# pharaofranz/frb-baseband

Measured on NVIDIA B200. Metric: input baseband GB/s (VDIF bytes, headers included) per B200, 2 Gbps 16x32 MHz 2-bit -> 8-bit Stokes I, higher is better.
Workload: dtype f32

## Files before the change

### frb-baseband_b200/csrc/b2f_api.cu

```cuda
#include <cuda_runtime.h>

#include <algorithm>
#include <cmath>
#include <cstdio>
#include <cstdlib>
#include <cstring>
#include <numeric>
#include <string>
#include <vector>

#define B2F_API_TU
#include "b2f_fused.cuh"
#include "b2f_generic.cuh"
#include "b2f_launch.h"

using namespace b2f;

namespace {

thread_local std::string g_err;

int fail(int code, const std::string& msg) {
    g_err = msg;
    return code;
// ... 57 lines not shown
    bool generic = false;
    int tsq = 1;
    float* d_Fk = nullptr;
    int64_t Fk_if_stride = 0, fk_pending = 0;
    int kgt_lg = 0;
    int kgt_cols = 0, kgt_rb = 0, kgt_col_ctas = 0, kgt_row_ctas = 0;
    bool carry_mode = false;
    float2 *d_tw_col = nullptr, *d_tw_row = nullptr;
    int nfilt_pos = 0, nfilt_neg = 0, keep = 0;
    int64_t step = 0;
    int64_t carry_len = 0;
    uint8_t* d_carry = nullptr;
    int bps = 1;
    bool smask = false;
    uint8_t* d_carry_mask = nullptr;
    float4* d_levels_stream = nullptr;
    int64_t levels_stride = 0;
    float2* d_spec = nullptr;
    float2* d_chirp = nullptr;
    uint8_t* d_out_stage[2]{};
    size_t out_stage_bytes[2]{};
    int path = 0;
    uint8_t* d_tstream = nullptr;  size_t tstream_stride = 0;
    int* d_fillflag = nullptr;     size_t fillflag_stride = 0;
    float* d_part = nullptr;       int64_t part_if_stride = 0;
    int Dp = 0;
    unsigned* d_fsync = nullptr;
    int f_grid = 0, f_lanes = 0, f_nslot = 3, f_lag = 2;
    bool f_aborted = false;
    float4* d_levels = nullptr;
    unsigned long long* d_fprof = nullptr;

    int64_t rows_base = 0;
    int64_t rows_off = 0;
    int64_t rows_held = 0;
    int64_t rows_produced = 0, rows_emitted = 0;
    bool stats_ready = false, flushed = false, have_base = false;
    int64_t rows_this_interval = 0;
    bool preset_stats = false;
    int64_t frames_pushed = 0;
    uint32_t base_sec0[B2F_MAX_IF]{}, base_fnum0[B2F_MAX_IF]{};
    int64_t last_nblk = 0, last_nframes = 0;
    unsigned long long blocks_dirty = 0;

    std::vector<TimedLaunch> pending;
    std::vector<std::pair<cudaEvent_t, cudaEvent_t>> ev_pool;
// ... 155 lines not shown
    body();
    CU(cudaGetLastError());
    return 0;
}

void free_plan(b2f_plan* pl) {
    if (!pl) return;
    cudaSetDevice(pl->prm.device);
    cudaDeviceSynchronize();
    for (int i = 0; i < 2; ++i) {
        if (pl->d_stage[i]) cudaFree(pl->d_stage[i]);
        if (pl->ev_stage_free[i]) cudaEventDestroy(pl->ev_stage_free[i]);
        if (pl->ev_h2d_done[i]) cudaEventDestroy(pl->ev_h2d_done[i]);
        if (pl->ev_out_free[i]) cudaEventDestroy(pl->ev_out_free[i]);
        if (pl->ev_kq_done[i]) cudaEventDestroy(pl->ev_kq_done[i]);
        if (pl->d_out_stage[i]) cudaFree(pl->d_out_stage[i]);
    }
    for (int i = 0; i < b2f_plan::kMarks; ++i)
        for (int k = 0; k < 3; ++k)
            if (pl->ev_mark[i][k]) cudaEventDestroy(pl->ev_mark[i][k]);
    void* bufs[] = {pl->d_compact, pl->d_wmask, pl->d_fstat, pl->d_blkdirty, pl->d_inter, pl->d_colsum,
                    pl->d_eps, pl->d_F, pl->d_mean, pl->d_scale, pl->d_partial, pl->d_tab_g, pl->d_tab_h,
                    pl->d_tab_w, pl->d_tab_r, pl->d_tab_beta, pl->d_counters, pl->d_carry, pl->d_spec, pl->d_chirp, pl->d_tw_col, pl->d_tw_row,
                    pl->d_tstream, pl->d_fillflag, pl->d_part, pl->d_fsync, pl->d_fprof, pl->d_levels, pl->d_carry_mask, pl->d_levels_stream};
    for (void* b : bufs)
        if (b) cudaFree(b);
    if (pl->d_Fk) cudaFree(pl->d_Fk);
    for (auto& t : pl->pending) { cudaEventDestroy(t.a); cudaEventDestroy(t.b); }
    for (auto& e : pl->ev_pool) { cudaEventDestroy(e.first); cudaEventDestroy(e.second); }
    if (pl->copy_stream) cudaStreamDestroy(pl->copy_stream);
    if (pl->d2h_stream) cudaStreamDestroy(pl->d2h_stream);
    if (pl->own_stream && pl->stream) cudaStreamDestroy(pl->stream);
    delete pl;
}

int init_state(b2f_plan* pl) {
    pl->rows_base = pl->rows_off = pl->rows_held = pl->rows_produced = pl->rows_emitted = 0;
    pl->stats_ready = pl->prm.keep_bandpass != 0 || pl->preset_stats;
    pl->flushed = false;
    pl->have_base = false;
    pl->frames_pushed = 0;
    pl->carry_len = 0;
    pl->fk_pending = 0;
    pl->blocks_dirty = 0;
    pl->last_nblk = pl->last_nframes = 0;
    pl->rows_this_interval = 0;
    pl->f_aborted = false;
// ... 258 lines not shown
    }
    if (pl->f_aborted) return fail(B2F_ECUDA, "fused channeliser: inter-warp wait timed out (results of this scan are invalid)");
    return 0;
}

int push_fused(b2f_plan* pl, const K0Params& k0, int64_t nframes, int64_t nblk) {
    const int nif = pl->prm.nif;
    const int64_t nbt = (int64_t)nif * nblk;
    int rc = 0;
    for (int i = 0; i < nif; ++i)
        if (reinterpret_cast<uintptr_t>(k0.frames[i]) & 15) return fail(B2F_EINVAL, "frames must be 16-byte aligned");
    K0HParams kh{};
    K0TParams kt{};
    for (int i = 0; i < nif; ++i) {
        kh.frames[i] = k0.frames[i]; kt.frames[i] = k0.frames[i];
        kh.base_sec[i] = k0.base_sec[i]; kh.base_fnum[i] = k0.base_fnum[i];
    }
    kh.fstat = pl->d_fstat; kh.fstat_stride = pl->fstat_stride; kh.counters = pl->d_counters;
    kh.nframes = nframes; kh.frame_bytes = pl->prm.frame_bytes; kh.header_bytes = pl->prm.header_bytes;
    kh.in_nbit = pl->prm.in_nbit; kh.fps = (int)pl->fps; kh.nif = nif;
    kt.fstat = pl->d_fstat; kt.fstat_stride = pl->fstat_stride;
    kt.fillflag = pl->d_fillflag; kt.fillflag_stride = pl->fillflag_stride;
    kt.tstream = pl->d_tstream; kt.tstream_if_stride = pl->tstream_stride; kt.counters = pl->d_counters;
    kt.nblk = (int)nblk; kt.nif = nif; kt.R = pl->R; kt.frame_bytes = pl->prm.frame_bytes;
    kt.header_bytes = pl->prm.header_bytes; kt.payload_bytes = (int)pl->payload; kt.mask_faults = pl->prm.mask_faults;
    CU(cudaMemsetAsync(pl->d_fillflag, 0, pl->fillflag_stride * nif * sizeof(int), pl->stream));
    rc = timed(pl, B2F_K_VALIDATE, [&] {
        const int64_t n = nframes * nif;
        k0h_headers<<<(unsigned)((n + 255) / 256), 256, 0, pl->stream>>>(kh);
        if (nblk > 0) {
            const int sc = std::min(64, pl->R);
            const int64_t units = nbt * (pl->R / sc);
            const unsigned grid = (unsigned)std::min<int64_t>(units, (int64_t)pl->num_sms * (sc == 64 ? 6 : 8));
            if (sc == 64) k0t_transpose<64><<<grid, 256, 0, pl->stream>>>(kt);
            else if (sc == 32) k0t_transpose<32><<<grid, 256, 0, pl->stream>>>(kt);
            else k0t_transpose<16><<<grid, 256, 0, pl->stream>>>(kt);
        }
    });
    if (rc) return rc;
    pl->launches++;
    if (nblk == 0) return 0;
    if (pl->d_levels) {
        KJParams kj{};
        for (int i = 0; i < nif; ++i) kj.frames[i] = k0.frames[i];
        kj.fstat = pl->d_fstat; kj.fstat_stride = pl->fstat_stride; kj.levels = pl->d_levels;
        kj.nblk = (int)nblk; kj.nif = nif; kj.R = pl->R; kj.frame_bytes = pl->prm.frame_bytes;
        kj.header_bytes = pl->prm.header_bytes; kj.payload_bytes = (int)pl->payload; kj.mask_faults = pl->prm.mask_faults;
        const int64_t nthreads = nbt * pl->R * 32;
        rc = timed(pl, B2F_K_VALIDATE, [&] { kj_ja98_levels<<<(unsigned)((nthreads + 255) / 256), 256, 0, pl->stream>>>(kj); });
        if (rc) return rc;
    }

    FParams fp{};
    fp.tstream = pl->d_tstream; fp.tstream_if_stride = pl->tstream_stride;
    fp.ring = pl->d_inter; fp.colsum = pl->d_colsum; fp.eps = pl->d_eps;
    fp.tab_h = pl->d_tab_h; fp.tab_w = pl->d_tab_w; fp.tab_beta = pl->d_tab_beta; fp.tab_r = pl->d_tab_r;
    const bool direct = pl->Dp == pl->D || pl->path == 1;
    fp.out = direct ? row_dst(pl) : pl->d_part;
    fp.out_if_stride = direct ? row_dst_stride(pl) : pl->part_if_stride;
    fp.out_row0 = direct ? row_dst_row0(pl) : 0;
    fp.Dp = pl->Dp; fp.nblk = (int)nblk; fp.nif = nif;
    fp.gb_begin = 0; fp.gb_end = nbt;
    fp.sync = pl->d_fsync; fp.abort_flag = pl->d_fsync + (size_t)pl->f_lanes * FS_STRIDE;
    fp.nslot = pl->f_nslot; fp.lag = pl->f_lag; fp.prof = pl->d_fprof; fp.levels = pl->d_levels;
    cudaError_t e = cudaSuccess;
    if (pl->path == 2) {
        CU(cudaMemsetAsync(pl->d_fsync, 0, (size_t)pl->f_lanes * FS_STRIDE * sizeof(unsigned), pl->stream));
        fp.phase = 0;
        rc = timed(pl, B2F_K_FUSED, [&] { e = b2f_launch_kf(pl->R, pl->prm.pol_mode, fp, pl->f_grid, 1, pl->stream, nullptr); });
        if (rc) return rc;
        if (e != cudaSuccess) return fail(B2F_ECUDA, std::string("fused channeliser launch: ") + cudaGetErrorString(e));
    } else {
        fp.phase = 1;
        rc = timed(pl, B2F_K_COLUMN, [&] { e = b2f_launch_kf(pl->R, B2F_POL_I, fp, pl->f_grid, 0, pl->stream, nullptr); });
        if (rc) return rc;
        if (e != cudaSuccess) return fail(B2F_ECUDA, std::string("column half launch: ") + cudaGetErrorString(e));
        rc = timed(pl, B2F_K_EPS, [&] {
// ... 279 lines not shown
    } else {
        CUB(cudaStreamCreateWithFlags(&pl->stream, cudaStreamNonBlocking));
        pl->own_stream = true;
    }
    CUB(cudaStreamCreateWithFlags(&pl->copy_stream, cudaStreamNonBlocking));
    CUB(cudaStreamCreateWithFlags(&pl->d2h_stream, cudaStreamNonBlocking));
    for (int i = 0; i < 2; ++i) {
        CUB(cudaEventCreateWithFlags(&pl->ev_stage_free[i], cudaEventDisableTiming));
        CUB(cudaEventCreateWithFlags(&pl->ev_h2d_done[i], cudaEventDisableTiming));
        CUB(cudaEventCreateWithFlags(&pl->ev_out_free[i], cudaEventDisableTiming));
        CUB(cudaEventCreateWithFlags(&pl->ev_kq_done[i], cudaEventDisableTiming));
    }
    const int nif = prm->nif;
    const int64_t nbt = (int64_t)nif * pl->chunk_blocks;
    pl->slot_bytes = W ? (int)spf : (prm->in_nbit == 8 ? payload : (int)spf);
    pl->compact_stride = (size_t)((pl->chunk_frames * (int64_t)pl->slot_bytes + (pl->carry_mode ? pl->M * pl->bps : 0) + 255) / 256 * 256);
    pl->wmask_stride = (size_t)((pl->chunk_frames * pl->groups_per_slot + (pl->smask ? pl->M * pl->bps / 32 : 0) + 255) / 256 * 256);
    pl->fstat_stride = (size_t)((pl->chunk_frames + 255) / 256 * 256);
    if (!pl->path) {
        CUB(cudaMalloc(&pl->d_compact, pl->compact_stride * nif));
        CUB(cudaMalloc(&pl->d_wmask, pl->wmask_stride * nif));
        CUB(cudaMalloc(&pl->d_blkdirty, (size_t)nbt));
    } else {
        pl->tstream_stride = (size_t)((pl->chunk_blocks * pl->M + 255) / 256 * 256);
        pl->fillflag_stride = (size_t)((pl->chunk_frames + 63) / 64 * 64);
        CUB(cudaMalloc(&pl->d_tstream, pl->tstream_stride * nif));
        CUB(cudaMalloc(&pl->d_fillflag, pl->fillflag_stride * nif * sizeof(int)));
        CUB(cudaMalloc(&pl->d_fsync, ((size_t)pl->f_lanes + 1) * FS_STRIDE * sizeof(unsigned)));
        CUB(cudaMemset(pl->d_fsync, 0, ((size_t)pl->f_lanes + 1) * FS_STRIDE * sizeof(unsigned)));
        if (prm->decode_mode == B2F_DECODE_JA98) CUB(cudaMalloc(&pl->d_levels, (size_t)nbt * R * sizeof(float4)));
        if (getenv("B2F_FUSED_PROF")) {
            CUB(cudaMalloc(&pl->d_fprof, (size_t)pl->f_grid * kFWarps * 8 * sizeof(unsigned long long)));
            CUB(cudaMemset(pl->d_fprof, 0, (size_t)pl->f_grid * kFWarps * 8 * sizeof(unsigned long long)));
        }
        if (pl->Dp < D && pl->path == 2) {
            pl->part_if_stride = pl->chunk_blocks * (L / pl->Dp) * nprod * pl->N;
            CUB(cudaMalloc(&pl->d_part, (size_t)pl->part_if_stride * nif * sizeof(float)));
        }
    }
    CUB(cudaMalloc(&pl->d_fstat, pl->fstat_stride * nif));
    int64_t inter_blocks = pl->batch_blocks > 0 ? std::min<int64_t>(pl->batch_blocks, nbt) : nbt;
    if (pl->path == 2) inter_blocks = (int64_t)pl->f_lanes * pl->f_nslot;
    CUB(cudaMalloc(&pl->d_inter, (size_t)inter_blocks * L * R * sizeof(float2)));
    CUB(cudaMalloc(&pl->d_colsum, (size_t)nbt * R * sizeof(float2)));
    CUB(cudaMalloc(&pl->d_eps, (size_t)nbt * pl->N * sizeof(float2)));
    pl->F_if_stride = pl->F_cap_rows * nprod * pl->N;
    CUB(cudaMalloc(&pl->d_F, (size_t)pl->F_if_stride * nif * sizeof(float)));
    if (tsq > 1) {
        pl->Fk_if_stride = (pl->chunk_blocks * pl->keep / D + tsq) * nprod * pl->N;
// ... 648 lines not shown
        const double fl = 2.0 * 64.0 * iters * (double)blocks * threads;
        if (rep >= 2) best = std::max(best, fl / (ms * 1e-3) / 1e12);
    }
    cudaEventDestroy(a);
    cudaEventDestroy(b);
    cudaFree(d);
    *tflops = best;
    return 0;
}

int b2f_debug_copy(b2f_plan* pl, int which, void* dst, size_t nbytes, size_t* needed) {
    if (!pl) return fail(B2F_EINVAL, "null plan");
    CU(cudaSetDevice(pl->prm.device));
    CU(cudaStreamSynchronize(pl->stream));
    const int nif = pl->prm.nif;
    const int64_t nbt = (int64_t)nif * pl->last_nblk;
    const void* src = nullptr;
    size_t n = 0;
    switch (which) {
        case 0:
            if (pl->path) { src = pl->d_tstream; n = pl->tstream_stride * nif; }
            else { src = pl->d_compact; n = pl->compact_stride * nif; }
            break;
        case 1: src = pl->d_wmask; n = pl->wmask_stride * nif; break;
        case 2: src = pl->d_fstat; n = pl->fstat_stride * nif; break;
        case 3: src = pl->d_blkdirty; n = (size_t)nbt; break;
        case 4: {
            int64_t nbk = pl->batch_blocks > 0 ? std::min<int64_t>(pl->batch_blocks, nbt) : nbt;
            if (pl->path == 2) nbk = (int64_t)pl->f_lanes * pl->f_nslot;
            src = pl->d_inter; n = (size_t)nbk * pl->L * pl->R * sizeof(float2); break;
        }
        case 5: src = pl->d_colsum; n = (size_t)nbt * pl->R * sizeof(float2); break;
        case 6: src = pl->d_eps; n = (size_t)nbt * pl->N * sizeof(float2); break;
        case 7: src = pl->d_F; n = (size_t)pl->F_if_stride * nif * sizeof(float); break;
        case 8: src = pl->d_fprof; n = (size_t)pl->f_grid * kFWarps * 8 * sizeof(unsigned long long); break;
        default: return fail(B2F_EINVAL, "which");
    }
    if (!src) return fail(B2F_EINVAL, "this buffer is not used by the plan's channeliser path");
    if (needed) *needed = n;
    if (!dst) return 0;
    CU(cudaMemcpy(dst, src, std::min(n, nbytes), cudaMemcpyDeviceToHost));
    return 0;
}

}
```

### frb-baseband_b200/csrc/b2f_fused.cuh

```cuda
#pragma once
#include "b2f_kernels.cuh"

namespace b2f {

constexpr int kFWarps = 16;
constexpr int kFThreads = kFWarps * 32;
constexpr unsigned kFSpinLimit = 1u << 22;

enum FSync { FS_COL = 0, FS_ROW = 1, FS_EPS = 2, FS_STRIDE = 32 };

template <int R> struct FShape;
template <> struct FShape<16>  { static constexpr int TR = 4,  PT = 4;  };
template <> struct FShape<32>  { static constexpr int TR = 4,  PT = 8;  };
template <> struct FShape<64>  { static constexpr int TR = 8,  PT = 8;  };
template <> struct FShape<128> { static constexpr int TR = 8,  PT = 16; };
#ifndef B2F_F256_TR
#define B2F_F256_TR 16
#endif
template <> struct FShape<256> { static constexpr int TR = B2F_F256_TR, PT = 256 / B2F_F256_TR; };
template <> struct FShape<512> { static constexpr int TR = 16, PT = 32; };

template <int R>
struct FGeo {
    static constexpr int TR = FShape<R>::TR, PT = FShape<R>::PT;
    static constexpr int N = R / 2, NPAIR = R / 2;
    static constexpr int RPW = 1024 / R;
    static constexpr int RW = 32 / TR;
    static constexpr int NPASS = RPW / RW;
    static constexpr int kPitch = R * 8 + (TR < 16 ? TR * 8 : 0);
    static constexpr int kXch = RW * TR * (PT + 1) * 8;
    static constexpr int kRowBuf = RPW * kPitch + (kXch > RW * kPitch ? kXch - RW * kPitch : 0);
    static constexpr int kColBuf = 16 * 34 * 16;
    static constexpr int kWarpBuf = ((kRowBuf > kColBuf ? kRowBuf : kColBuf) + 127) / 128 * 128;
    static constexpr int kOffW4 = 0;
    static constexpr int kOffLut = kOffW4 + 8 * 32 * 16;
    static constexpr int kOffTw = kOffLut + 256;
    static constexpr int kOffH = kOffTw + R * 8;
    static constexpr int kOffBuf = (kOffH + kFWarps * 512 + 127) / 128 * 128;
    static constexpr size_t kBytes = (size_t)kOffBuf + (size_t)kFWarps * kWarpBuf;
};

struct FParams {
    const uint8_t* tstream;
    size_t tstream_if_stride;
    float2* ring;
    float2* colsum;
    float2* eps;
    const float2 *tab_h, *tab_w, *tab_beta, *tab_r;
    float* out;
    int64_t out_if_stride;
    int64_t out_row0;
    int Dp;
    int nblk, nif;
    int64_t gb_begin, gb_end;
    unsigned* sync;
    unsigned* abort_flag;
    int phase;
    int nslot;
    int lag;
    const float4* levels;
    unsigned long long* prof;
};

__device__ __forceinline__ unsigned ld_acquire_u32(const unsigned* p) {
    unsigned v;
    asm volatile("ld.acquire.gpu.global.u32 %0, [%1];" : "=r"(v) : "l"(p) : "memory");
    return v;
// ... 27 lines not shown
    }
}
__device__ __forceinline__ void warp_arrive_relaxed(unsigned* ctr, int lane) {
    __syncwarp();
    if (lane == 0) asm volatile("red.relaxed.gpu.global.add.u32 [%0], 1;" ::"l"(ctr) : "memory");
}
__device__ __forceinline__ float2 ldcg_f2(const float2* p) {
    float2 v;
    asm volatile("ld.global.cg.v2.f32 {%0, %1}, [%2];" : "=f"(v.x), "=f"(v.y) : "l"(p) : "memory");
    return v;
}
__device__ __forceinline__ uint4 ldg_stream16(const void* p) {
    uint4 v;
    asm volatile("ld.global.nc.L1::no_allocate.v4.u32 {%0, %1, %2, %3}, [%4];"
                 : "=r"(v.x), "=r"(v.y), "=r"(v.z), "=r"(v.w) : "l"(p));
    return v;
}

__device__ __forceinline__ float2 f_ja98(float2 v, float4 lv) {
    const float ax = fabsf(v.x), ay = fabsf(v.y);
    return make_float2(ax == 0.f ? 0.f : copysignf(ax > 2.f ? lv.y : lv.x, v.x), ay == 0.f ? 0.f : copysignf(ay > 2.f ? lv.w : lv.z, v.y));
}

template <int R, bool JA98>
__device__ __forceinline__ void f_col_front(const uint4 rawA, const uint4 rawB, float4* xb, const float4* s_w4,
                                            const uint8_t* s_lut, const float4* s_h4w, const int lane, float2* colsum_n1,
                                            const float4* levels_blk) {
    const int item = lane >> 1, col = lane & 1;
    {
        float2 vA[16], vB[16];
        const uint32_t wa[4] = {rawA.x, rawA.y, rawA.z, rawA.w}, wb[4] = {rawB.x, rawB.y, rawB.z, rawB.w};
#pragma unroll
        for (int r = 0; r < 16; ++r) {
            const uint32_t ia = __byte_perm(wa[r >> 2], 0u, 0x4440 + (r & 3));
            const uint32_t ib = __byte_perm(wb[r >> 2], 0u, 0x4440 + (r & 3));
            vA[r] = *reinterpret_cast<const float2*>(s_lut + ia);
            vB[r] = *reinterpret_cast<const float2*>(s_lut + ib);
        }
        if (JA98) {
#pragma unroll
            for (int r = 0; r < 16; ++r) {
                const int rowA = 32 * r + item;
                vA[r] = f_ja98(vA[r], __ldg(levels_blk + ((rowA * R) >> 9)));
                vB[r] = f_ja98(vB[r], __ldg(levels_blk + (((rowA + 16) * R) >> 9)));
            }
        }
        fft_inreg<16, false>(vA);
        fft_inreg<16, false>(vB);
#pragma unroll
        for (int qp = 0; qp < 8; ++qp) {
            const float4 ta = s_w4[qp * 32 + item], tb = s_w4[qp * 32 + item + 16];
            if (qp) vA[2 * qp] = cmul(vA[2 * qp], make_float2(ta.x, ta.y));
            vA[2 * qp + 1] = cmul(vA[2 * qp + 1], make_float2(ta.z, ta.w));
            if (qp) vB[2 * qp] = cmul(vB[2 * qp], make_float2(tb.x, tb.y));
// ... 199 lines not shown
    __syncwarp();
}

template <int R, int MODE, bool JA98>
__global__ void __launch_bounds__(kFThreads, 1) kf_fused(const FParams p) {
    using G = FGeo<R>;
    extern __shared__ __align__(128) uint8_t kf_smem[];
    float4* s_w4 = reinterpret_cast<float4*>(kf_smem + G::kOffW4);
    uint8_t* s_lut = kf_smem + G::kOffLut;
    float2* s_tw = reinterpret_cast<float2*>(kf_smem + G::kOffTw);
    const int tid = threadIdx.x, lane = tid & 31, warp = tid >> 5;
    float4* s_h4w = reinterpret_cast<float4*>(kf_smem + G::kOffH + warp * 512);
    uint8_t* wbuf = kf_smem + G::kOffBuf + (size_t)warp * G::kWarpBuf;

    for (int i = tid; i < 8 * 32; i += kFThreads) {
        const int qp = i >> 5, l = i & 31;
        const float2 w0 = p.tab_w[l * 16 + 2 * qp], w1 = p.tab_w[l * 16 + 2 * qp + 1];
        s_w4[i] = make_float4(w0.x, w0.y, w1.x, w1.y);
    }
    if (tid < 32) {
        const int c0 = tid & 3, c1 = (tid >> 2) & 3;
        const float m0 = (c0 == 0 || c0 == 3) ? kLevHi : kLevLo;
        const float m1 = (c1 == 0 || c1 == 3) ? kLevHi : kLevLo;
        if (tid <= 16)
            reinterpret_cast<float2*>(s_lut)[tid] = tid < 16 ? make_float2((c0 & 2) ? m0 : -m0, (c1 & 2) ? m1 : -m1) : make_float2(0.f, 0.f);
    }
    for (int i = tid; i < G::PT * G::TR; i += kFThreads) s_tw[i] = p.tab_r[i];

    const int gw = blockIdx.x * kFWarps + warp;
    const int nl = (int)(gridDim.x * kFWarps) / G::NPAIR;
    const int lam = gw % nl, pr = gw / nl;
    const bool active = pr < G::NPAIR;
    const int item = lane >> 1, col = lane & 1;
    const int n1 = 2 * (active ? pr : 0) + col;
    {
        const int pp = lane >> 1;
        const float2 h0 = p.tab_h[pp * R + n1], h1 = p.tab_h[(pp + 16) * R + n1];
        s_h4w[pp * 2 + col] = make_float4(h0.x, h0.y, h1.x, h1.y);
    }
    float2 betaS[4];
#pragma unroll
    for (int k = 0; k < 4; ++k) betaS[k] = p.tab_beta[(size_t)(item * 4 + k) * R + n1];
    __syncthreads();
    if (!active) return;

    const int64_t nb = p.gb_end - p.gb_begin;
    const int64_t M = (int64_t)R * kL;
    unsigned* sy = p.sync + (size_t)lam * FS_STRIDE;
    const int phase = p.phase, ns = p.nslot;
    const int lag = phase == 0 ? p.lag : 0;

    auto raw_ptr = [&](int64_t lb) {
        const int64_t gb = p.gb_begin + lb;
        const int ifi = (int)(gb / p.nblk);
        const int64_t blk = gb % p.nblk;
        return p.tstream + ifi * p.tstream_if_stride + blk * M + (size_t)pr * 1024 + (size_t)lane * 16;
    };
    uint4 rawA = make_uint4(0, 0, 0, 0), rawB = rawA;
    if (phase != 2 && lam < nb) {
        const uint8_t* q = raw_ptr(lam);
        rawA = ldg_stream16(q);
        rawB = ldg_stream16(q + 512);
    }

#ifdef B2F_KF_PROF
    unsigned long long tacc[8] = {0, 0, 0, 0, 0, 0, 0, 0};
    long long tprev = clock64();
    auto tick = [&](int k) {
        if (p.prof) {
            const long long t = clock64();
            tacc[k] += (unsigned long long)(t - tprev);
            tprev = t;
        }
    };
#else
    auto tick = [](int) {};
#endif
    bool col_pending = false;
#pragma unroll 1
    for (int i = 0;; ++i) {
        const int64_t lbc = (int64_t)i * nl + lam;
        const int64_t lbr = lbc - (int64_t)lag * nl;
        const int64_t lbe = lbc - nl;
        const bool vc = phase != 2 && lbc < nb;
        const bool vr = phase != 1 && lbr >= 0 && lbr < nb;
        const bool ve = phase == 0 && lbe >= 0 && lbe < nb && pr == (i % G::NPAIR);
// ... 2 lines not shown
        unsigned c_col = 0, c_row = 0, c_eps = 0;
        if (phase == 0) {
            c_col = ld_relaxed_u32(sy + FS_COL);
            c_eps = ld_relaxed_u32(sy + FS_EPS);
            c_row = ld_relaxed_u32(sy + FS_ROW);
        }
        tick(7);
        if (vr) {
            const int64_t gb = p.gb_begin + lbr;
            const int64_t slot = phase == 0 ? (int64_t)lam * ns + ((i - lag) % ns) : lbr;
            if (phase == 0) {
                if (c_col < (unsigned)(G::NPAIR * (i - lag + 1)) &&
                    !warp_wait_ge(sy + FS_COL, (unsigned)(G::NPAIR * (i - lag + 1)), p.abort_flag, lane)) return;
                if (c_eps < (unsigned)(i - lag + 1) && !warp_wait_ge(sy + FS_EPS, (unsigned)(i - lag + 1), p.abort_flag, lane)) return;
            }
            tick(3);
            f_row_load<R>(p.ring + slot * M, pr * G::RPW, wbuf, lane);
            cp_async_wait<0>();
            __syncwarp();
            tick(4);
        }
        if (col_pending) { warp_arrive(sy + FS_COL, lane); col_pending = false; }
        if (vr && phase == 0) warp_arrive_relaxed(sy + FS_ROW, lane);
        if (vc && i > 0 && phase != 1) {
            const uint8_t* q = raw_ptr(lbc);
            rawA = ldg_stream16(q);
            rawB = ldg_stream16(q + 512);
        }
        tick(5);
        if (vr) {
            const int64_t gb = p.gb_begin + lbr;
            f_row_compute<R, MODE>(p, wbuf, s_tw, p.eps + gb * G::N, gb, pr * G::RPW, lane);
            __syncwarp();
            tick(6);
        }
        if (ve) {
            if (!warp_wait_ge(sy + FS_COL, (unsigned)(G::NPAIR * i), p.abort_flag, lane)) return;
            const int64_t gb = p.gb_begin + lbe;
            f_eps<R>(p.colsum + gb * R, p.eps + gb * G::N, wbuf, s_tw, lane);
            __syncwarp();
            if (lane == 0) {
                __threadfence();
                atomicMax(sy + FS_EPS, (unsigned)i);
            }
            tick(3);
        }
        if (vc) {
            const int64_t gb = p.gb_begin + lbc;
            const int64_t slot = phase == 0 ? (int64_t)lam * ns + (i % ns) : lbc;
            f_col_front<R, JA98>(rawA, rawB, reinterpret_cast<float4*>(wbuf), s_w4, s_lut, s_h4w, lane, p.colsum + gb * R + n1,
                                 JA98 ? p.levels + gb * R : nullptr);
            tick(0);
            if (phase == 0 && i >= ns && c_row < (unsigned)(G::NPAIR * (i - ns + 1))) {
                if (!warp_wait_ge(sy + FS_ROW, (unsigned)(G::NPAIR * (i - ns + 1)), p.abort_flag, lane)) return;
            }
            tick(1);
            if (phase == 1 && lbc + nl < nb) {
                const uint8_t* q = raw_ptr(lbc + nl);
                rawA = ldg_stream16(q);
                rawB = ldg_stream16(q + 512);
            }
            f_col_back<R>(reinterpret_cast<const float4*>(wbuf), betaS, lane, p.ring + slot * M + (size_t)pr * 32);
            col_pending = phase == 0;
            tick(2);
        }
        if (lag < 2 && col_pending) { warp_arrive(sy + FS_COL, lane); col_pending = false; }
    }
    if (col_pending) warp_arrive(sy + FS_COL, lane);
#ifdef B2F_KF_PROF
    if (p.prof && lane == 0) {
#pragma unroll
        for (int k = 0; k < 8; ++k) atomicAdd(&p.prof[(size_t)gw * 8 + k], tacc[k]);
    }
#endif
}

struct KTParams {
    const float2* inter;
    const float2* eps;
    const float2* tab_r;
    float* F; int64_t F_if_stride; int64_t row0;
    int nblk, nif, D;
    int64_t nb;
};
// ... 160 lines not shown
            }
#pragma unroll
            for (int pp = 0; pp < 8; ++pp)
#pragma unroll
                for (int c = 0; c < NPROD; ++c) acc[pp][c] = 0.f;
        }
    }
}

struct K0HParams {
    const uint8_t* frames[B2F_MAX_IF];
    uint8_t* fstat; size_t fstat_stride;
    unsigned long long* counters;
    int64_t nframes;
    int frame_bytes, header_bytes, in_nbit, fps, nif;
    uint32_t base_sec[B2F_MAX_IF], base_fnum[B2F_MAX_IF];
};

struct K0TParams {
    const uint8_t* frames[B2F_MAX_IF];
    const uint8_t* fstat; size_t fstat_stride;
    int* fillflag; size_t fillflag_stride;
    uint8_t* tstream; size_t tstream_if_stride;
    unsigned long long* counters;
    int nblk, nif, R, frame_bytes, header_bytes, payload_bytes, mask_faults;
};

#ifdef B2F_API_TU
static __global__ void k0h_headers(const K0HParams p) {
    const int64_t i = blockIdx.x * (int64_t)blockDim.x + threadIdx.x;
    const bool in = i < p.nframes * p.nif;
    int bad = 0, inv = 0, mis = 0, alive = 0;
    if (in) {
        const int ifi = (int)(i / p.nframes);
        const int64_t f = i % p.nframes;
        const uint4 h = *reinterpret_cast<const uint4*>(p.frames[ifi] + f * p.frame_bytes);
        const bool invalid = (h.x >> 31) != 0;
        const bool badh = ((h.z & 0xFFFFFFu) * 8u != (uint32_t)p.frame_bytes) || ((int)((h.w >> 26) & 31u) + 1 != p.in_nbit) ||
                          ((int)((h.x >> 30) & 1u) != (p.header_bytes == 16 ? 1 : 0));
        const int64_t tslot = ((int64_t)(h.x & 0x3FFFFFFFu) - (int64_t)p.base_sec[ifi]) * p.fps +
                              ((int64_t)(h.y & 0xFFFFFFu) - (int64_t)p.base_fnum[ifi]);
        p.fstat[ifi * p.fstat_stride + f] = (invalid || badh) ? 2 : 1;
        bad = badh;
        inv = !badh && invalid;
        alive = !badh && !invalid;
        mis = tslot != f;
    }
    const unsigned nb = __popc(__ballot_sync(0xffffffffu, bad)), ni = __popc(__ballot_sync(0xffffffffu, inv));
    const unsigned nm = __popc(__ballot_sync(0xffffffffu, mis)), na = __popc(__ballot_sync(0xffffffffu, alive));
    if ((threadIdx.x & 31) == 0) {
        if (nb) atomicAdd(&p.counters[C_BADHDR], (unsigned long long)nb);
        if (ni) atomicAdd(&p.counters[C_INVALID], (unsigned long long)ni);
        if (nm) atomicAdd(&p.counters[C_MISPLACED], (unsigned long long)nm);
        if (na) atomicAdd(&p.counters[C_OK], (unsigned long long)na);
    }
}

template <int SC>
static __global__ void __launch_bounds__(256) k0t_transpose(const K0TParams p) {
    constexpr int PB = SC / 2;
    constexpr int NW = PB / 4;
    constexpr int PITCH = SC + 8;
    __shared__ __align__(16) uint8_t s_exp[kL * PITCH];
    const int tid = threadIdx.x;
    const int R = p.R, nstrip = R / SC;
    const int64_t M = (int64_t)R * kL;
    const int64_t nunits = (int64_t)p.nif * p.nblk * nstrip;
    unsigned long long nfill_total = 0;
    uint32_t w[2][NW];
    uint8_t dead[2];
    int64_t fr[2];
    int fif = 0;
    auto load_unit = [&](int64_t u) {
        const int strip = (int)(u % nstrip);
        const int64_t gb = u / nstrip;
        const int ifi = (int)(gb / p.nblk);
        const int64_t blk = gb % p.nblk;
        const uint8_t* frames = p.frames[ifi];
        fif = ifi;
#pragma unroll
        for (int k = 0; k < 2; ++k) {
            const int row = tid + 256 * k;
            const int64_t pb = (blk * M + (int64_t)R * row + (int64_t)strip * SC) >> 1;
            const int64_t f = pb / p.payload_bytes;
            const int off = (int)(pb - f * p.payload_bytes);
            const uint8_t* src = frames + f * p.frame_bytes + p.header_bytes + off;
            if (NW >= 4) {
#pragma unroll
                for (int v = 0; v < NW / 4; ++v) {
                    const uint4 x = ldg_stream16(src + 16 * v);
                    w[k][(4 * v) % NW] = x.x; w[k][(4 * v + 1) % NW] = x.y; w[k][(4 * v + 2) % NW] = x.z; w[k][(4 * v + 3) % NW] = x.w;
                }
            } else {
                const uint2 x = *reinterpret_cast<const uint2*>(src);
                w[k][0] = x.x; w[k][1 % NW] = x.y;
            }
            dead[k] = p.fstat[ifi * p.fstat_stride + f];
            fr[k] = f;
        }
    };
    if (blockIdx.x < nunits) load_unit(blockIdx.x);
    for (int64_t u = blockIdx.x; u < nunits; u += gridDim.x) {
        const int strip = (int)(u % nstrip);
        const int64_t gb = u / nstrip;
        const int ifi = (int)(gb / p.nblk);
        const int64_t blk = gb % p.nblk;
#pragma unroll
        for (int k = 0; k < 2; ++k) {
            const int row = tid + 256 * k;
            const bool isdead = dead[k] == 2;
            unsigned fm = 0;
#pragma unroll
            for (int j = 0; j < NW; ++j) fm |= (unsigned)(w[k][j] == kFillWord) << j;
            if (fm && !isdead) {
                nfill_total += __popc(fm);
                if (p.mask_faults && atomicExch(&p.fillflag[fif * p.fillflag_stride + fr[k]], 1) == 0) {
                    atomicAdd(&p.counters[C_FILLFRAMES], 1ull);
                    atomicAdd(&p.counters[C_OK], ~0ull);
                }
            }
            const unsigned mask = !p.mask_faults ? 0u : (isdead ? 0xFFFFu : fm);
            uint2* d = reinterpret_cast<uint2*>(s_exp + row * PITCH);
#pragma unroll
            for (int j = 0; j < NW; ++j) d[j] = expand_word_2bit(w[k][j], (mask >> j) & 1);
        }
        __syncthreads();
        if (u + gridDim.x < nunits) load_unit(u + gridDim.x);
        {
            const int lane = tid & 31, wrp = tid >> 5;
            const int item = lane & 15;
            const int half = wrp >> 2;
            const int c8 = (wrp & 3) * 2 + (lane >> 4);
            uint8_t* tb = p.tstream + ifi * p.tstream_if_stride + blk * M;
            if (c8 < SC / 8) {
                uint32_t o[8][4];
#pragma unroll
                for (int g = 0; g < 4; ++g) {
                    uint2 a[4];
#pragma unroll
                    for (int j = 0; j < 4; ++j)
                        a[j] = *reinterpret_cast<const uint2*>(s_exp + (32 * (4 * g + j) + item + 16 * half) * PITCH + 8 * c8);
                    {
                        const uint32_t t0 = __byte_perm(a[0].x, a[1].x, 0x5140), t1 = __byte_perm(a[2].x, a[3].x, 0x5140);
                        const uint32_t t2 = __byte_perm(a[0].x, a[1].x, 0x7362), t3 = __byte_perm(a[2].x, a[3].x, 0x7362);
                        o[0][g] = __byte_perm(t0, t1, 0x5410);
                        o[1][g] = __byte_perm(t0, t1, 0x7632);
                        o[2][g] = __byte_perm(t2, t3, 0x5410);
                        o[3][g] = __byte_perm(t2, t3, 0x7632);
                    }
                    {
                        const uint32_t t0 = __byte_perm(a[0].y, a[1].y, 0x5140), t1 = __byte_perm(a[2].y, a[3].y, 0x5140);
                        const uint32_t t2 = __byte_perm(a[0].y, a[1].y, 0x7362), t3 = __byte_perm(a[2].y, a[3].y, 0x7362);
                        o[4][g] = __byte_perm(t0, t1, 0x5410);
                        o[5][g] = __byte_perm(t0, t1, 0x7632);
                        o[6][g] = __byte_perm(t2, t3, 0x5410);
                        o[7][g] = __byte_perm(t2, t3, 0x7632);
                    }
                }
                const bool odd = lane & 1;
#pragma unroll
                for (int pp = 0; pp < 4; ++pp) {
                    uint32_t rcv[4];
#pragma unroll
                    for (int k = 0; k < 4; ++k) rcv[k] = __shfl_xor_sync(0xffffffffu, odd ? o[2 * pp][k] : o[2 * pp + 1][k], 1);
                    const int pair = strip * (SC / 2) + 4 * c8 + pp;
                    uint8_t* pb = tb + (size_t)(pair * 2 + half) * 32 * 16;
                    *reinterpret_cast<uint4*>(pb + (2 * (item & ~1) + (int)odd) * 16) =
                        odd ? make_uint4(rcv[0], rcv[1], rcv[2], rcv[3]) : make_uint4(o[2 * pp][0], o[2 * pp][1], o[2 * pp][2], o[2 * pp][3]);
                    *reinterpret_cast<uint4*>(pb + (2 * (item | 1) + (int)odd) * 16) =
                        odd ? make_uint4(o[2 * pp + 1][0], o[2 * pp + 1][1], o[2 * pp + 1][2], o[2 * pp + 1][3]) : make_uint4(rcv[0], rcv[1], rcv[2], rcv[3]);
                }
            }
        }
        __syncthreads();
    }
    for (int m = 16; m; m >>= 1) nfill_total += __shfl_xor_sync(0xffffffffu, nfill_total, m);
    if ((tid & 31) == 0 && nfill_total) atomicAdd(&p.counters[C_FILLWORDS], nfill_total);
}

struct KJParams {
    const uint8_t* frames[B2F_MAX_IF];
    const uint8_t* fstat; size_t fstat_stride;
    float4* levels;
    int nblk, nif, R, frame_bytes, header_bytes, payload_bytes, mask_faults;
};
static __global__ void kj_ja98_levels(const KJParams p) {
    const int lane = threadIdx.x & 31;
    const int64_t w = (blockIdx.x * (int64_t)blockDim.x + threadIdx.x) >> 5;
    const int64_t nwin = (int64_t)p.nif * p.nblk * p.R;
    if (w >= nwin) return;
    const int ifi = (int)(w / ((int64_t)p.nblk * p.R));
    const int64_t wi = w % ((int64_t)p.nblk * p.R);
    unsigned lowP = 0, lowQ = 0, nval = 0;
#pragma unroll
    for (int k = 0; k < 2; ++k) {
        const int64_t pb = wi * 256 + (lane + 32 * k) * 4;
        const int64_t f = pb / p.payload_bytes;
// ... 50 lines not shown
```

Before: 111.0.

## Keep transposed stream in packed 2-bit form with sparse mask plane

```diff
diff --git a/frb-baseband_b200/csrc/b2f_api.cu b/frb-baseband_b200/csrc/b2f_api.cu
--- a/frb-baseband_b200/csrc/b2f_api.cu
+++ b/frb-baseband_b200/csrc/b2f_api.cu
@@ -103,6 +103,7 @@
     size_t out_stage_bytes[2]{};
     int path = 0;
     uint8_t* d_tstream = nullptr;  size_t tstream_stride = 0;
+    uint8_t* d_mflag = nullptr;    uint32_t* d_mplane = nullptr;
     int* d_fillflag = nullptr;     size_t fillflag_stride = 0;
     float* d_part = nullptr;       int64_t part_if_stride = 0;
     int Dp = 0;
@@ -304,7 +305,7 @@
     void* bufs[] = {pl->d_compact, pl->d_wmask, pl->d_fstat, pl->d_blkdirty, pl->d_inter, pl->d_colsum,
                     pl->d_eps, pl->d_F, pl->d_mean, pl->d_scale, pl->d_partial, pl->d_tab_g, pl->d_tab_h,
                     pl->d_tab_w, pl->d_tab_r, pl->d_tab_beta, pl->d_counters, pl->d_carry, pl->d_spec, pl->d_chirp, pl->d_tw_col, pl->d_tw_row,
-                    pl->d_tstream, pl->d_fillflag, pl->d_part, pl->d_fsync, pl->d_fprof, pl->d_levels, pl->d_carry_mask, pl->d_levels_stream};
+                    pl->d_tstream, pl->d_mflag, pl->d_mplane, pl->d_fillflag, pl->d_part, pl->d_fsync, pl->d_fprof, pl->d_levels, pl->d_carry_mask, pl->d_levels_stream};
     for (void* b : bufs)
         if (b) cudaFree(b);
     if (pl->d_Fk) cudaFree(pl->d_Fk);
@@ -609,6 +610,7 @@
     kt.fstat = pl->d_fstat; kt.fstat_stride = pl->fstat_stride;
     kt.fillflag = pl->d_fillflag; kt.fillflag_stride = pl->fillflag_stride;
     kt.tstream = pl->d_tstream; kt.tstream_if_stride = pl->tstream_stride; kt.counters = pl->d_counters;
+    kt.mflag = pl->d_mflag; kt.mplane = pl->d_mplane;
     kt.nblk = (int)nblk; kt.nif = nif; kt.R = pl->R; kt.frame_bytes = pl->prm.frame_bytes;
     kt.header_bytes = pl->prm.header_bytes; kt.payload_bytes = (int)pl->payload; kt.mask_faults = pl->prm.mask_faults;
     CU(cudaMemsetAsync(pl->d_fillflag, 0, pl->fillflag_stride * nif * sizeof(int), pl->stream));
@@ -616,9 +618,9 @@
         const int64_t n = nframes * nif;
         k0h_headers<<<(unsigned)((n + 255) / 256), 256, 0, pl->stream>>>(kh);
         if (nblk > 0) {
-            const int sc = std::min(64, pl->R);
+            const int sc = k0t_strip_cols(pl->R);
             const int64_t units = nbt * (pl->R / sc);
-            const unsigned grid = (unsigned)std::min<int64_t>(units, (int64_t)pl->num_sms * (sc == 64 ? 6 : 8));
+            const unsigned grid = (unsigned)std::min<int64_t>(units, (int64_t)pl->num_sms * kK0TCtasPerSM);
             if (sc == 64) k0t_transpose<64><<<grid, 256, 0, pl->stream>>>(kt);
             else if (sc == 32) k0t_transpose<32><<<grid, 256, 0, pl->stream>>>(kt);
             else k0t_transpose<16><<<grid, 256, 0, pl->stream>>>(kt);
@@ -640,6 +642,7 @@
 
     FParams fp{};
     fp.tstream = pl->d_tstream; fp.tstream_if_stride = pl->tstream_stride;
+    fp.mflag = pl->d_mflag; fp.mplane = pl->d_mplane;
     fp.ring = pl->d_inter; fp.colsum = pl->d_colsum; fp.eps = pl->d_eps;
     fp.tab_h = pl->d_tab_h; fp.tab_w = pl->d_tab_w; fp.tab_beta = pl->d_tab_beta; fp.tab_r = pl->d_tab_r;
     const bool direct = pl->Dp == pl->D || pl->path == 1;
@@ -965,9 +968,11 @@
         CUB(cudaMalloc(&pl->d_wmask, pl->wmask_stride * nif));
         CUB(cudaMalloc(&pl->d_blkdirty, (size_t)nbt));
     } else {
-        pl->tstream_stride = (size_t)((pl->chunk_blocks * pl->M + 255) / 256 * 256);
+        pl->tstream_stride = (size_t)((pl->chunk_blocks * pl->M / 2 + 255) / 256 * 256);
         pl->fillflag_stride = (size_t)((pl->chunk_frames + 63) / 64 * 64);
         CUB(cudaMalloc(&pl->d_tstream, pl->tstream_stride * nif));
+        CUB(cudaMalloc(&pl->d_mflag, (size_t)nbt * (R / k0t_strip_cols(R))));
+        CUB(cudaMalloc(&pl->d_mplane, (size_t)nbt * (R / 2) * 32 * sizeof(uint32_t)));
         CUB(cudaMalloc(&pl->d_fillflag, pl->fillflag_stride * nif * sizeof(int)));
         CUB(cudaMalloc(&pl->d_fsync, ((size_t)pl->f_lanes + 1) * FS_STRIDE * sizeof(unsigned)));
         CUB(cudaMemset(pl->d_fsync, 0, ((size_t)pl->f_lanes + 1) * FS_STRIDE * sizeof(unsigned)));
@@ -1662,7 +1667,10 @@
             if (pl->path) { src = pl->d_tstream; n = pl->tstream_stride * nif; }
             else { src = pl->d_compact; n = pl->compact_stride * nif; }
             break;
-        case 1: src = pl->d_wmask; n = pl->wmask_stride * nif; break;
+        case 1:
+            if (pl->path) { src = pl->d_mflag; n = (size_t)nbt * (pl->R / k0t_strip_cols(pl->R)); }
+            else { src = pl->d_wmask; n = pl->wmask_stride * nif; }
+            break;
         case 2: src = pl->d_fstat; n = pl->fstat_stride * nif; break;
         case 3: src = pl->d_blkdirty; n = (size_t)nbt; break;
         case 4: {
diff --git a/frb-baseband_b200/csrc/b2f_fused.cuh b/frb-baseband_b200/csrc/b2f_fused.cuh
--- a/frb-baseband_b200/csrc/b2f_fused.cuh
+++ b/frb-baseband_b200/csrc/b2f_fused.cuh
@@ -40,9 +40,14 @@
     static constexpr size_t kBytes = (size_t)kOffBuf + (size_t)kFWarps * kWarpBuf;
 };
 
+constexpr int k0t_strip_cols(int R) { return R < 64 ? R : 64; }
+constexpr int kK0TCtasPerSM = 3;
+
 struct FParams {
     const uint8_t* tstream;
     size_t tstream_if_stride;
+    const uint8_t* mflag;
+    const uint32_t* mplane;
     float2* ring;
     float2* colsum;
     float2* eps;
@@ -116,14 +121,30 @@
     return make_float2(ax == 0.f ? 0.f : copysignf(ax > 2.f ? lv.y : lv.x, v.x), ay == 0.f ? 0.f : copysignf(ay > 2.f ? lv.w : lv.z, v.y));
 }
 
+__device__ __forceinline__ uint32_t mask_bytes4(uint32_t m4) { return (((m4 & 15u) * 0x00204081u) & 0x01010101u) << 7; }
+
 template <int R, bool JA98>
-__device__ __forceinline__ void f_col_front(const uint4 rawA, const uint4 rawB, float4* xb, const float4* s_w4,
-                                            const uint8_t* s_lut, const float4* s_h4w, const int lane, float2* colsum_n1,
-                                            const float4* levels_blk) {
+__device__ __forceinline__ void f_col_front(const uint4 rawA, const uint4 rawB, const bool mflag, const uint32_t* mword,
+                                            float4* xb, const float4* s_w4, const uint8_t* s_lut, const float4* s_h4w,
+                                            const int lane, float2* colsum_n1, const float4* levels_blk) {
     const int item = lane >> 1, col = lane & 1;
     {
         float2 vA[16], vB[16];
-        const uint32_t wa[4] = {rawA.x, rawA.y, rawA.z, rawA.w}, wb[4] = {rawB.x, rawB.y, rawB.z, rawB.w};
+        const int rot = col ? 31 : 3;
+        uint32_t wa[4] = {rawA.x, rawA.y, rawA.z, rawA.w}, wb[4] = {rawB.x, rawB.y, rawB.z, rawB.w};
+#pragma unroll
+        for (int k = 0; k < 4; ++k) {
+            wa[k] = __funnelshift_l(wa[k], wa[k], rot) & 0x78787878u;
+            wb[k] = __funnelshift_l(wb[k], wb[k], rot) & 0x78787878u;
+        }
+        if (mflag) {
+            const uint32_t m = __ldg(mword);
+#pragma unroll
+            for (int k = 0; k < 4; ++k) {
+                wa[k] |= mask_bytes4(m >> (4 * k));
+                wb[k] |= mask_bytes4(m >> (16 + 4 * k));
+            }
+        }
 #pragma unroll
         for (int r = 0; r < 16; ++r) {
             const uint32_t ia = __byte_perm(wa[r >> 2], 0u, 0x4440 + (r & 3));
@@ -369,8 +390,7 @@
         const int c0 = tid & 3, c1 = (tid >> 2) & 3;
         const float m0 = (c0 == 0 || c0 == 3) ? kLevHi : kLevLo;
         const float m1 = (c1 == 0 || c1 == 3) ? kLevHi : kLevLo;
-        if (tid <= 16)
-            reinterpret_cast<float2*>(s_lut)[tid] = tid < 16 ? make_float2((c0 & 2) ? m0 : -m0, (c1 & 2) ? m1 : -m1) : make_float2(0.f, 0.f);
+        reinterpret_cast<float2*>(s_lut)[tid] = tid < 16 ? make_float2((c0 & 2) ? m0 : -m0, (c1 & 2) ? m1 : -m1) : make_float2(0.f, 0.f);
     }
     for (int i = tid; i < G::PT * G::TR; i += kFThreads) s_tw[i] = p.tab_r[i];
 
@@ -397,18 +417,19 @@
     const int phase = p.phase, ns = p.nslot;
     const int lag = phase == 0 ? p.lag : 0;
 
-    auto raw_ptr = [&](int64_t lb) {
+    constexpr int kStripPairs = k0t_strip_cols(R) / 2;
+    uint4 rawA = make_uint4(0, 0, 0, 0), rawB = rawA;
+    bool mflag = false;
+    auto load_raw = [&](int64_t lb) {
         const int64_t gb = p.gb_begin + lb;
         const int ifi = (int)(gb / p.nblk);
         const int64_t blk = gb % p.nblk;
-        return p.tstream + ifi * p.tstream_if_stride + blk * M + (size_t)pr * 1024 + (size_t)lane * 16;
+        const uint8_t* q = p.tstream + ifi * p.tstream_if_stride + blk * (M / 2) + (size_t)pr * 512 + (size_t)item * 16;
+        rawA = ldg_stream16(q);
+        rawB = ldg_stream16(q + 256);
+        mflag = __ldg(p.mflag + gb * (R / k0t_strip_cols(R)) + pr / kStripPairs) != 0;
     };
-    uint4 rawA = make_uint4(0, 0, 0, 0), rawB = rawA;
-    if (phase != 2 && lam < nb) {
-        const uint8_t* q = raw_ptr(lam);
-        rawA = ldg_stream16(q);
-        rawB = ldg_stream16(q + 512);
-    }
+    if (phase != 2 && lam < nb) load_raw(lam);
 
 #ifdef B2F_KF_PROF
     unsigned long long tacc[8] = {0, 0, 0, 0, 0, 0, 0, 0};
@@ -457,11 +478,7 @@
         }
         if (col_pending) { warp_arrive(sy + FS_COL, lane); col_pending = false; }
         if (vr && phase == 0) warp_arrive_relaxed(sy + FS_ROW, lane);
-        if (vc && i > 0 && phase != 1) {
-            const uint8_t* q = raw_ptr(lbc);
-            rawA = ldg_stream16(q);
-            rawB = ldg_stream16(q + 512);
-        }
+        if (vc && i > 0 && phase != 1) load_raw(lbc);
         tick(5);
         if (vr) {
             const int64_t gb = p.gb_begin + lbr;
@@ -483,18 +500,14 @@
         if (vc) {
             const int64_t gb = p.gb_begin + lbc;
             const int64_t slot = phase == 0 ? (int64_t)lam * ns + (i % ns) : lbc;
-            f_col_front<R, JA98>(rawA, rawB, reinterpret_cast<float4*>(wbuf), s_w4, s_lut, s_h4w, lane, p.colsum + gb * R + n1,
-                                 JA98 ? p.levels + gb * R : nullptr);
+            f_col_front<R, JA98>(rawA, rawB, mflag, p.mplane + (gb * G::NPAIR + pr) * 32 + lane, reinterpret_cast<float4*>(wbuf), s_w4,
+                                 s_lut, s_h4w, lane, p.colsum + gb * R + n1, JA98 ? p.levels + gb * R : nullptr);
             tick(0);
             if (phase == 0 && i >= ns && c_row < (unsigned)(G::NPAIR * (i - ns + 1))) {
                 if (!warp_wait_ge(sy + FS_ROW, (unsigned)(G::NPAIR * (i - ns + 1)), p.abort_flag, lane)) return;
             }
             tick(1);
-            if (phase == 1 && lbc + nl < nb) {
-                const uint8_t* q = raw_ptr(lbc + nl);
-                rawA = ldg_stream16(q);
-                rawB = ldg_stream16(q + 512);
-            }
+            if (phase == 1 && lbc + nl < nb) load_raw(lbc + nl);
             f_col_back<R>(reinterpret_cast<const float4*>(wbuf), betaS, lane, p.ring + slot * M + (size_t)pr * 32);
             col_pending = phase == 0;
             tick(2);
@@ -701,6 +714,8 @@
     const uint8_t* fstat; size_t fstat_stride;
     int* fillflag; size_t fillflag_stride;
     uint8_t* tstream; size_t tstream_if_stride;
+    uint8_t* mflag;
+    uint32_t* mplane;
     unsigned long long* counters;
     int nblk, nif, R, frame_bytes, header_bytes, payload_bytes, mask_faults;
 };
@@ -736,27 +751,31 @@
 }
 
 template <int SC>
-static __global__ void __launch_bounds__(256) k0t_transpose(const K0TParams p) {
+static __global__ void __launch_bounds__(256, kK0TCtasPerSM) k0t_transpose(const K0TParams p) {
     constexpr int PB = SC / 2;
     constexpr int NW = PB / 4;
-    constexpr int PITCH = SC + 8;
-    __shared__ __align__(16) uint8_t s_exp[kL * PITCH];
+    constexpr int NP = SC / 2;
+    constexpr int PITCH = NW + 1;
+    __shared__ uint32_t s_raw[kL * PITCH];
+    __shared__ uint32_t s_mask[NP * 16];
     const int tid = threadIdx.x;
     const int R = p.R, nstrip = R / SC;
     const int64_t M = (int64_t)R * kL;
     const int64_t nunits = (int64_t)p.nif * p.nblk * nstrip;
     unsigned long long nfill_total = 0;
-    uint32_t w[2][NW];
-    uint8_t dead[2];
-    int64_t fr[2];
-    int fif = 0;
-    auto load_unit = [&](int64_t u) {
+    struct Stage {
+        uint32_t w[2][NW];
+        uint8_t dead[2];
+        int64_t fr[2];
+        int fif;
+    } st0, st1;
+    auto load_unit = [&](int64_t u, Stage& S) {
         const int strip = (int)(u % nstrip);
         const int64_t gb = u / nstrip;
         const int ifi = (int)(gb / p.nblk);
         const int64_t blk = gb % p.nblk;
         const uint8_t* frames = p.frames[ifi];
-        fif = ifi;
+        S.fif = ifi;
 #pragma unroll
         for (int k = 0; k < 2; ++k) {
             const int row = tid + 256 * k;
@@ -768,90 +787,94 @@
 #pragma unroll
                 for (int v = 0; v < NW / 4; ++v) {
                     const uint4 x = ldg_stream16(src + 16 * v);
-                    w[k][(4 * v) % NW] = x.x; w[k][(4 * v + 1) % NW] = x.y; w[k][(4 * v + 2) % NW] = x.z; w[k][(4 * v + 3) % NW] = x.w;
+                    S.w[k][(4 * v) % NW] = x.x; S.w[k][(4 * v + 1) % NW] = x.y; S.w[k][(4 * v + 2) % NW] = x.z; S.w[k][(4 * v + 3) % NW] = x.w;
                 }
             } else {
                 const uint2 x = *reinterpret_cast<const uint2*>(src);
-                w[k][0] = x.x; w[k][1 % NW] = x.y;
-            }
-            dead[k] = p.fstat[ifi * p.fstat_stride + f];
-            fr[k] = f;
+                S.w[k][0] = x.x; S.w[k][1 % NW] = x.y;
+            }
+            S.dead[k] = p.fstat[ifi * p.fstat_stride + f];
+            S.fr[k] = f;
         }
     };
-    if (blockIdx.x < nunits) load_unit(blockIdx.x);
-    for (int64_t u = blockIdx.x; u < nunits; u += gridDim.x) {
+    for (int i = tid; i < NP * 16; i += 256) s_mask[i] = 0;
+    const int64_t g = gridDim.x;
+    auto process_unit = [&](int64_t u, Stage& S) {
         const int strip = (int)(u % nstrip);
         const int64_t gb = u / nstrip;
         const int ifi = (int)(gb / p.nblk);
         const int64_t blk = gb % p.nblk;
+        int dirty = 0;
 #pragma unroll
         for (int k = 0; k < 2; ++k) {
             const int row = tid + 256 * k;
-            const bool isdead = dead[k] == 2;
+            const bool isdead = S.dead[k] == 2;
             unsigned fm = 0;
 #pragma unroll
-            for (int j = 0; j < NW; ++j) fm |= (unsigned)(w[k][j] == kFillWord) << j;
+            for (int j = 0; j < NW; ++j) fm |= (unsigned)(S.w[k][j] == kFillWord) << j;
             if (fm && !isdead) {
                 nfill_total += __popc(fm);
-                if (p.mask_faults && atomicExch(&p.fillflag[fif * p.fillflag_stride + fr[k]], 1) == 0) {
+                if (p.mask_faults && atomicExch(&p.fillflag[S.fif * p.fillflag_stride + S.fr[k]], 1) == 0) {
                     atomicAdd(&p.counters[C_FILLFRAMES], 1ull);
                     atomicAdd(&p.counters[C_OK], ~0ull);
                 }
             }
-            const unsigned mask = !p.mask_faults ? 0u : (isdead ? 0xFFFFu : fm);
-            uint2* d = reinterpret_cast<uint2*>(s_exp + row * PITCH);
-#pragma unroll
-            for (int j = 0; j < NW; ++j) d[j] = expand_word_2bit(w[k][j], (mask >> j) & 1);
+#pragma unroll
+            for (int j = 0; j < NW; ++j) s_raw[row * PITCH + j] = S.w[k][j];
+            const unsigned mask = !p.mask_faults ? 0u : (isdead ? (1u << NW) - 1 : fm);
+            if (mask) {
+                dirty = 1;
+                const uint32_t bit = 1u << ((row >> 5) + 16 * ((row >> 4) & 1));
+#pragma unroll
+                for (int j = 0; j < NW; ++j)
+                    if ((mask >> j) & 1)
+#pragma unroll
+                        for (int q = 0; q < 4; ++q) atomicOr(&s_mask[(4 * j + q) * 16 + (row & 15)], bit);
+            }
+        }
+        dirty = __syncthreads_or(dirty);
+        if (u + 2 * g < nunits) load_unit(u + 2 * g, S);
+        {
+            const int item = tid & 15, half = (tid >> 4) & 1, c4 = tid >> 5;
+            if (c4 < NW) {
+                uint32_t a[16];
+#pragma unroll
+                for (int r = 0; r < 16; ++r) a[r] = s_raw[(32 * r + 16 * half + item) * PITCH + c4];
+                uint32_t o[4][4];
+#pragma unroll
+                for (int g = 0; g < 4; ++g) {
+                    const uint32_t t0 = __byte_perm(a[4 * g], a[4 * g + 1], 0x5140), t1 = __byte_perm(a[4 * g + 2], a[4 * g + 3], 0x5140);
+                    const uint32_t t2 = __byte_perm(a[4 * g], a[4 * g + 1], 0x7362), t3 = __byte_perm(a[4 * g + 2], a[4 * g + 3], 0x7362);
+                    o[0][g] = __byte_perm(t0, t1, 0x5410);
+                    o[1][g] = __byte_perm(t0, t1, 0x7632);
+                    o[2][g] = __byte_perm(t2, t3, 0x5410);
+                    o[3][g] = __byte_perm(t2, t3, 0x7632);
+                }
+                uint8_t* tb = p.tstream + ifi * p.tstream_if_stride + blk * (M / 2);
+#pragma unroll
+                for (int j = 0; j < 4; ++j) {
+                    const int pair = strip * NP + 4 * c4 + j;
+                    *reinterpret_cast<uint4*>(tb + ((size_t)(pair * 2 + half) * 16 + item) * 16) = make_uint4(o[j][0], o[j][1], o[j][2], o[j][3]);
+                }
+            }
+        }
+        if (tid == 0) p.mflag[gb * nstrip + strip] = (uint8_t)dirty;
+        if (dirty) {
+            uint2* mp = reinterpret_cast<uint2*>(p.mplane + (gb * (R / 2) + strip * NP) * 32);
+            for (int i = tid; i < NP * 16; i += 256) {
+                const uint32_t m = s_mask[i];
+                s_mask[i] = 0;
+                mp[i] = make_uint2(m, m);
+            }
         }
         __syncthreads();
-        if (u + gridDim.x < nunits) load_unit(u + gridDim.x);
-        {
-            const int lane = tid & 31, wrp = tid >> 5;
-            const int item = lane & 15;
-            const int half = wrp >> 2;
-            const int c8 = (wrp & 3) * 2 + (lane >> 4);
-            uint8_t* tb = p.tstream + ifi * p.tstream_if_stride + blk * M;
-            if (c8 < SC / 8) {
-                uint32_t o[8][4];
-#pragma unroll
-                for (int g = 0; g < 4; ++g) {
-                    uint2 a[4];
-#pragma unroll
-                    for (int j = 0; j < 4; ++j)
-                        a[j] = *reinterpret_cast<const uint2*>(s_exp + (32 * (4 * g + j) + item + 16 * half) * PITCH + 8 * c8);
-                    {
-                        const uint32_t t0 = __byte_perm(a[0].x, a[1].x, 0x5140), t1 = __byte_perm(a[2].x, a[3].x, 0x5140);
-                        const uint32_t t2 = __byte_perm(a[0].x, a[1].x, 0x7362), t3 = __byte_perm(a[2].x, a[3].x, 0x7362);
-                        o[0][g] = __byte_perm(t0, t1, 0x5410);
-                        o[1][g] = __byte_perm(t0, t1, 0x7632);
-                        o[2][g] = __byte_perm(t2, t3, 0x5410);
-                        o[3][g] = __byte_perm(t2, t3, 0x7632);
-                    }
-                    {
-                        const uint32_t t0 = __byte_perm(a[0].y, a[1].y, 0x5140), t1 = __byte_perm(a[2].y, a[3].y, 0x5140);
-                        const uint32_t t2 = __byte_perm(a[0].y, a[1].y, 0x7362), t3 = __byte_perm(a[2].y, a[3].y, 0x7362);
-                        o[4][g] = __byte_perm(t0, t1, 0x5410);
-                        o[5][g] = __byte_perm(t0, t1, 0x7632);
-                        o[6][g] = __byte_perm(t2, t3, 0x5410);
-                        o[7][g] = __byte_perm(t2, t3, 0x7632);
-                    }
-                }
-                const bool odd = lane & 1;
-#pragma unroll
-                for (int pp = 0; pp < 4; ++pp) {
-                    uint32_t rcv[4];
-#pragma unroll
-                    for (int k = 0; k < 4; ++k) rcv[k] = __shfl_xor_sync(0xffffffffu, odd ? o[2 * pp][k] : o[2 * pp + 1][k], 1);
-                    const int pair = strip * (SC / 2) + 4 * c8 + pp;
-                    uint8_t* pb = tb + (size_t)(pair * 2 + half) * 32 * 16;
-                    *reinterpret_cast<uint4*>(pb + (2 * (item & ~1) + (int)odd) * 16) =
-                        odd ? make_uint4(rcv[0], rcv[1], rcv[2], rcv[3]) : make_uint4(o[2 * pp][0], o[2 * pp][1], o[2 * pp][2], o[2 * pp][3]);
-                    *reinterpret_cast<uint4*>(pb + (2 * (item | 1) + (int)odd) * 16) =
-                        odd ? make_uint4(o[2 * pp + 1][0], o[2 * pp + 1][1], o[2 * pp + 1][2], o[2 * pp + 1][3]) : make_uint4(rcv[0], rcv[1], rcv[2], rcv[3]);
-                }
-            }
-        }
-        __syncthreads();
+    };
+    if (blockIdx.x < nunits) load_unit(blockIdx.x, st0);
+    if (blockIdx.x + g < nunits) load_unit(blockIdx.x + g, st1);
+    __syncthreads();
+    for (int64_t u = blockIdx.x; u < nunits; u += 2 * g) {
+        process_unit(u, st0);
+        if (u + g < nunits) process_unit(u + g, st1);
     }
     for (int m = 16; m; m >>= 1) nfill_total += __shfl_xor_sync(0xffffffffu, nfill_total, m);
     if ((tid & 31) == 0 && nfill_total) atomicAdd(&p.counters[C_FILLWORDS], nfill_total);
```

After: 113.1, median of 6. 1.02x the previous value.
